# Scalsol/mega.pytorch

Hardware: AMD Instinct MI355X
Metric: frames/sec MEGA R-101 inference, 1000x600 VID clip (higher is better)
Workload: dtype bf16

## Files before the change

### include/mega_hip.h

```cpp
#ifndef MEGA_HIP_H
#define MEGA_HIP_H

#include <stddef.h>

#ifdef __cplusplus
extern "C" {
#endif

#define MEGA_F32 0
#define MEGA_BF16 1
#define MEGA_F16 2

#define MEGA_OK 0
#define MEGA_ERR_ARG 1
#define MEGA_ERR_LAUNCH 2
#define MEGA_ERR_WS 3
#define MEGA_ERR_LIMIT 4

int mega_conv2d_nhwc(const void* in, const void* w, const float* scale, const float* bias, const void* residual,
                     void* out, int N, int H, int W, int Cin, int Cout, int R, int S, int stride, int pad, int dil,
                     int relu, int ldo, int ldr, int in_dtype, int out_dtype, void* stream);
int mega_conv2d_nhwc_tile(int M, int Cout, int K);
int mega_conv2d_nhwc_plan(int M, int Cout, int K, int in_dtype);
int mega_conv2d_nhwc_plan_ex(int N, int H, int W, int Cin, int Cout, int R, int S, int stride, int pad, int dil, int ldo,
                             int has_residual, int in_dtype, int out_dtype);

size_t mega_conv2d_nhwc_workspace_bytes(int M, int Cout, int K);
int mega_conv2d_nhwc_ws(const void* in, const void* w, const float* scale, const float* bias, const void* residual,
                        void* out, int N, int H, int W, int Cin, int Cout, int R, int S, int stride, int pad, int dil,
                        int relu, int ldo, int ldr, int in_dtype, int out_dtype, void* ws, size_t ws_bytes, void* stream);

int mega_stem_conv_bn_relu(const float* in, const float* w_tap64, const float* scale, const float* bias, void* out,
                           int N, int H, int W, int out_dtype, void* stream);
int mega_stem_conv_bn_relu_bf16(const float* in, const void* w_n176_bf16, const float* scale, const float* bias,
                                void* out, int N, int H, int W, void* stream);
int mega_stem_conv_bn_relu_bf16_u8(const void* frames_u8, const void* w_n176_bf16, const float* scale, const float* bias,
                                   void* out, int N, int H, int W, float mean0, float mean1, float mean2, int to_bgr,
                                   void* stream);

int mega_stem_pool_dt(const void* in, int u8, const void* w_n176, const float* scale, const float* bias, void* out, int N,
                      int H, int W, float mean0, float mean1, float mean2, int to_bgr, int dtype, void* stream);

int mega_maxpool3x3s2_nhwc(const void* in, void* out, int N, int H, int W, int C, int dtype, void* stream);

int mega_avgpool2x2_ceil_nhwc(const void* in, void* out, int N, int H, int W, int C, int dtype, void* stream);

int mega_roi_align_fwd(const void* feat, const float* rois, void* out, int K, int C, int H, int W,
                       float spatial_scale, int pooled_h, int pooled_w, int sampling_ratio, int in_nhwc,
                       int out_nhwc, int dtype, int out_dtype, void* stream);

size_t mega_nms_full_workspace_bytes(int n);
int mega_nms(const float* dets, const float* scores, int n, float thr, int strict_gt, long long* keep_out,
             int* keep_cnt, void* ws, size_t ws_bytes, void* stream);

size_t mega_nms_workspace_bytes(int P, int nmax);
int mega_nms_sorted(const float* boxes, const int* counts, const unsigned char* valid, const int* order, int P,
                    int nmax, float thr, int strict_gt, int max_keep, int* keep_pos, int* keep_cnt,
                    unsigned char* flags, void* ws, size_t ws_bytes, void* stream);

size_t mega_rpn_select_workspace_bytes(int B, int pre_nms_top_n);
int mega_rpn_select_idx(const float* rpn_out, const float* cell_anchors, int B, int Hf, int Wf, int A, int ldc,
                        int anchor_stride, int pre_nms_top_n, int post_nms_top_n, float nms_thresh, int strict_gt,
                        float min_size, float im_w, float im_h, float* proposals, float* prop_scores, int* prop_cnt,
                        int* prop_index, void* ws, size_t ws_bytes, void* stream);

size_t mega_postprocess_workspace_bytes(int R, int NC);
int mega_postprocess(const float* logits, const float* deltas, const float* props, const int* nprop, int R, int NC,
                     float wx, float wy, float ww, float wh, float im_w, float im_h, float score_thresh,
                     float nms_thresh, int strict_gt, int max_det, float* out_boxes, float* out_scores,
                     long long* out_labels, int* out_cnt, float* probs_out, void* ws, size_t ws_bytes,
                     void* stream);

size_t mega_postprocess_batched_workspace_bytes(int B, int R, int NC);
int mega_postprocess_batched(const float* logits, const float* deltas, const float* props, const int* nprop, int B,
                             int R, int NC, float wx, float wy, float ww, float wh, float im_w, float im_h,
                             float score_thresh, float nms_thresh, int strict_gt, int max_det, float* out_boxes,
                             float* out_scores, long long* out_labels, int* out_cnt, float* probs_out, void* ws,
                             size_t ws_bytes, void* stream);

int mega_postprocess_candidates_batched(const float* logits, const float* deltas, const float* props, const int* nprop,
                                        int B, int R, int NC, float wx, float wy, float ww, float wh, float im_w,
                                        float im_h, float score_thresh, float* cboxes, float* cscores, void* stream);

size_t mega_bbox_aug_merge_workspace_bytes(int F, int K, int R, int NC);
int mega_bbox_aug_merge(const float* cboxes, const float* cscores, int F, int K, int R, int NC, const int* view_w,
                        const int* view_h, const int* view_flip, float score_thresh, float nms_thresh, int strict_gt,
                        int max_det, float* out_boxes, float* out_scores, long long* out_labels, int* out_cnt, void* ws,
                        size_t ws_bytes, void* stream);

size_t mega_soft_merge_workspace_bytes(int F, int K, int R, int NC);
int mega_soft_merge(const float* cboxes, const float* cscores, int F, int K, int R, int NC, const int* view_w,
                    const int* view_h, const int* view_flip, float score_thresh, float nms_thresh, int strict_gt,
                    int soft_method, float sigma, int vote, float vote_thresh, int vote_scoring, int max_det,
                    float* out_boxes, float* out_scores, long long* out_labels, int* out_cnt, void* ws, size_t ws_bytes,
// ... 159 lines not shown
```

### mega/pytorch_amd/_lib.py

```python
import ctypes
import os

HERE = os.path.dirname(os.path.abspath(__file__))
LIB_PATH = os.path.join(HERE, "libmega_hip.so")

c_int, c_float, c_void_p, c_size_t = ctypes.c_int, ctypes.c_float, ctypes.c_void_p, ctypes.c_size_t
c_longlong = ctypes.c_longlong

_ERR = {1: "bad argument", 2: "kernel launch failure", 3: "workspace too small", 4: "kernel loop bound exceeded"}

SIGNATURES = {
    "mega_conv2d_nhwc": (c_int, [c_void_p] * 6 + [c_int] * 15 + [c_void_p]),
    "mega_conv2d_nhwc_ws": (c_int, [c_void_p] * 6 + [c_int] * 15 + [c_void_p, c_size_t, c_void_p]),
    "mega_conv2d_nhwc_workspace_bytes": (c_size_t, [c_int] * 3),
    "mega_stem_conv_bn_relu": (c_int, [c_void_p] * 5 + [c_int] * 4 + [c_void_p]),
    "mega_stem_conv_bn_relu_bf16": (c_int, [c_void_p] * 5 + [c_int] * 3 + [c_void_p]),
    "mega_stem_conv_bn_relu_bf16_u8": (c_int, [c_void_p] * 5 + [c_int] * 3 + [c_float] * 3 + [c_int, c_void_p]),
    "mega_stem_pool_dt": (c_int, [c_void_p, c_int] + [c_void_p] * 4 + [c_int] * 3 + [c_float] * 3 + [c_int, c_int, c_void_p]),
    "mega_maxpool3x3s2_nhwc": (c_int, [c_void_p] * 2 + [c_int] * 5 + [c_void_p]),
    "mega_avgpool2x2_ceil_nhwc": (c_int, [c_void_p] * 2 + [c_int] * 5 + [c_void_p]),
    "mega_roi_align_fwd": (c_int, [c_void_p] * 3 + [c_int] * 4 + [c_float] + [c_int] * 7 + [c_void_p]),
    "mega_nms_full_workspace_bytes": (c_size_t, [c_int]),
    "mega_nms": (c_int, [c_void_p, c_void_p, c_int, c_float, c_int, c_void_p, c_void_p, c_void_p, c_size_t, c_void_p]),
    "mega_nms_workspace_bytes": (c_size_t, [c_int, c_int]),
    "mega_nms_sorted": (c_int, [c_void_p] * 4 + [c_int, c_int, c_float, c_int, c_int] + [c_void_p] * 4 +
                        [c_size_t, c_void_p]),
    "mega_rpn_select_workspace_bytes": (c_size_t, [c_int, c_int]),
    "mega_rpn_select_idx": (c_int, [c_void_p, c_void_p] + [c_int] * 8 + [c_float, c_int, c_float, c_float, c_float] +
                            [c_void_p] * 5 + [c_size_t, c_void_p]),
    "mega_postprocess_workspace_bytes": (c_size_t, [c_int, c_int]),
    "mega_postprocess": (c_int, [c_void_p] * 4 + [c_int, c_int] + [c_float] * 8 + [c_int, c_int] + [c_void_p] * 6 +
                         [c_size_t, c_void_p]),
    "mega_postprocess_batched_workspace_bytes": (c_size_t, [c_int, c_int, c_int]),
    "mega_postprocess_batched": (c_int, [c_void_p] * 4 + [c_int, c_int, c_int] + [c_float] * 8 + [c_int, c_int] +
                                 [c_void_p] * 6 + [c_size_t, c_void_p]),
    "mega_postprocess_candidates_batched": (c_int, [c_void_p] * 4 + [c_int] * 3 + [c_float] * 7 + [c_void_p] * 3),
    "mega_bbox_aug_merge_workspace_bytes": (c_size_t, [c_int] * 4),
    "mega_bbox_aug_merge": (c_int, [c_void_p, c_void_p] + [c_int] * 4 + [c_void_p] * 3 + [c_float, c_float, c_int, c_int] +
                            [c_void_p] * 5 + [c_size_t, c_void_p]),
    "mega_soft_merge_workspace_bytes": (c_size_t, [c_int] * 4),
    "mega_soft_merge": (c_int, [c_void_p, c_void_p] + [c_int] * 4 + [c_void_p] * 3 +
                        [c_float, c_float, c_int, c_int, c_float, c_int, c_float, c_int, c_int] + [c_void_p] * 5 +
                        [c_size_t, c_void_p]),
    "mega_position_logits": (c_int, [c_void_p] * 6 + [c_int] * 4 + [c_void_p]),
    "mega_relation_attention_splits": (c_int, [c_int, c_int, c_int]),
    "mega_relation_attention_workspace_bytes": (c_size_t, [c_int, c_int, c_int]),
    "mega_relation_attention": (c_int, [c_void_p, c_int, c_void_p, c_int, c_void_p, c_int, c_void_p, c_int,
                                        c_void_p, c_int, c_void_p, c_void_p, c_int, c_int, c_int, c_int, c_float,
                                        c_int, c_void_p, c_size_t, c_void_p]),
    "mega_relation_attention_batched": (c_int, [c_void_p, c_int, c_int, c_float, c_int, c_void_p]),
    "mega_position_logits_tiled_dt": (c_int, [c_void_p] * 6 + [c_int] * 3 + [c_void_p]),
    "mega_position_logits_tiled_batched_dt": (c_int, [c_void_p, c_int, c_void_p, c_void_p, c_void_p, c_int, c_void_p]),
    "mega_relation_attention_tiled_pos_dt": (c_int, [c_void_p, c_int, c_void_p, c_int, c_void_p, c_int, c_void_p,
                                                     c_void_p, c_int, c_void_p, c_void_p, c_int, c_int, c_int, c_int,
                                                     c_float, c_int, c_void_p, c_size_t, c_void_p]),
    "mega_conv2d_nhwc_tile": (c_int, [c_int] * 3),
    "mega_conv2d_nhwc_plan": (c_int, [c_int] * 4),
    "mega_conv2d_nhwc_plan_ex": (c_int, [c_int] * 14),
    "mega_preprocess_frames": (c_int, [c_void_p, c_void_p] + [c_int] * 3 + [c_float] * 3 + [c_int, c_void_p]),
    "mega_dff_warp_scale": (c_int, [c_void_p] * 4 + [c_int] * 4 + [c_void_p]),
    "mega_fgfa_pair_taps": (c_int, [c_void_p, c_longlong, c_void_p, c_longlong, c_void_p, c_void_p] + [c_int] * 4 + [c_void_p]),
    "mega_resize_bilinear_u8": (c_int, [c_void_p] * 3 + [c_int] * 5 + [c_void_p, c_void_p, c_int, c_void_p, c_void_p,
                                                                      c_int, c_void_p]),
    "mega_resize_bilinear_u8_flip": (c_int, [c_void_p] * 3 + [c_int] * 5 + [c_void_p, c_void_p, c_int, c_void_p,
                                                                           c_void_p, c_int, c_int, c_void_p]),
    "mega_fgfa_warp_aggregate": (c_int, [c_void_p] * 4 + [c_int] * 7 + [c_void_p]),
    "mega_fgfa_warp_aggregate_ring": (c_int, [c_void_p] * 4 + [c_int] * 5 + [c_void_p, c_int, c_void_p]),
    "mega_copy_segments": (c_int, [c_void_p, c_int, c_void_p]),
    "mega_bottleneck64_fwd_dt": (c_int, [c_void_p] * 11 + [c_int] * 4 + [c_void_p]),
    "mega_bottleneck64_ds_fwd_dt": (c_int, [c_void_p] * 14 + [c_int] * 4 + [c_void_p]),
    "mega_cast_f32_to_half": (c_int, [c_void_p, c_void_p, c_size_t, c_int, c_void_p]),
# ... 65 lines not shown
```

### mega/pytorch_amd/csrc/spatial.hip

```cpp
#include "common.h"

namespace {

constexpr int ST_T = 16;
constexpr int ST_P = ST_T * 2 + 5;
constexpr int ST_PW = ST_P + 1;

template <typename OT>
__global__ __launch_bounds__(256) void stem_conv_kernel(const float* __restrict__ in, const float* __restrict__ w,
                                                        const float* __restrict__ scale,
                                                        const float* __restrict__ bias, OT* __restrict__ out, int N,
                                                        int H, int W, int Ho, int Wo) {
  __shared__ float patch[3][ST_P][ST_PW];
  const int tid = threadIdx.x;
  const int n = blockIdx.z;
  const int oy0 = blockIdx.y * ST_T, ox0 = blockIdx.x * ST_T;
  const int iy0 = oy0 * 2 - 3, ix0 = ox0 * 2 - 3;
  for (int e = tid; e < 3 * ST_P * ST_P; e += 256) {
    const int c = e / (ST_P * ST_P);
    const int rem = e - c * ST_P * ST_P;
    const int y = rem / ST_P, x = rem - y * ST_P;
    const int iy = iy0 + y, ix = ix0 + x;
    float v = 0.f;
    if ((unsigned)iy < (unsigned)H && (unsigned)ix < (unsigned)W) v = in[((size_t)(n * 3 + c) * H + iy) * W + ix];
// ... 506 lines not shown
  f32x16_t acc[2][2];
#pragma unroll
  for (int i = 0; i < 2; ++i)
#pragma unroll
    for (int j = 0; j < 2; ++j)
#pragma unroll
      for (int r = 0; r < 16; ++r) acc[i][j][r] = 0.f;
#pragma unroll
  for (int ks = 0; ks < SM_K / 16; ++ks) {
    uint4 a[2], b[2];
#pragma unroll
    for (int i = 0; i < 2; ++i) {
      const unsigned* base = reinterpret_cast<const unsigned*>(
          patch + (2 * (2 * wave + i)) * SM_PS + 2 * p + (half ? stem_group_off(2 * ks + 1) : stem_group_off(2 * ks)));
      a[i] = make_uint4(base[0], base[1], base[2], base[3]);
    }
#pragma unroll
    for (int j = 0; j < 2; ++j)
      b[j] = *reinterpret_cast<const uint4*>(&wl[(j * 32 + p) * SM_WS + ks * 16 + half * 8]);
#pragma unroll
    for (int i = 0; i < 2; ++i)
#pragma unroll
      for (int j = 0; j < 2; ++j)
        acc[i][j] = __builtin_amdgcn_mfma_f32_32x32x16_bf16(__builtin_bit_cast(bf16x8_t, a[i]),
                                                            __builtin_bit_cast(bf16x8_t, b[j]), acc[i][j], 0, 0, 0);
  }
  __syncthreads();
#pragma unroll
  for (int j = 0; j < 2; ++j) {
    const int ch = j * 32 + p;
    const float sc = scale[ch], bi = bias[ch];
#pragma unroll
    for (int i = 0; i < 2; ++i) {
#pragma unroll
      for (int r = 0; r < 16; ++r) {
        const int px = (r & 3) + 8 * (r >> 2) + 4 * half;
        *reinterpret_cast<unsigned short*>(smem + ((2 * wave + i) * SM_TX + px) * SM_OUT_PS + ch * 2) =
            (bf16_t)(f32_to_bf16(fmaxf(acc[i][j][r] * sc + bi, 0.f)) & 0x7fffu);
      }
    }
  }
  __syncthreads();
#pragma unroll
  for (int i = 0; i < SM_TY * SM_TX * 8 / 256; ++i) {
    const int v = tid + 256 * i;
    const int pl = v >> 3, cv = v & 7;
    const int oy = oy0 + pl / SM_TX, ox = ox0 + pl % SM_TX;
    if (oy < Ho && ox < Wo)
      *reinterpret_cast<uint4*>(out + (((size_t)n * Ho + oy) * Wo + ox) * 64 + cv * 8) =
          *reinterpret_cast<const uint4*>(smem + pl * SM_OUT_PS + cv * 16);
  }
}

constexpr int SP_PY = 4, SP_PX = 16;
constexpr int SP_TY = 2 * SP_PY + 1, SP_TX = 2 * SP_PX + 1;
constexpr int SP_NPIX = SP_TY * SP_TX;
constexpr int SP_NBLK = (SP_NPIX + 31) / 32;
constexpr int SP_PH = 2 * SP_TY + 5, SP_PW = 2 * SP_TX + 5, SP_PS = 72;
static_assert(SP_PW + 1 <= SP_PS, "the zero-weight 8th tap reads one column past the patch");

__host__ __device__ constexpr int sp_group_off(int g) {
  const int gg = g < 21 ? g : 20;
  return (gg / 7) * (SP_PH * SP_PS) + (gg % 7) * SP_PS;
}

template <bool U8, typename HT = bf16_t>
__global__ __launch_bounds__(256, 3) void stem_pool_kernel(const void* __restrict__ in_, const bf16_t* __restrict__ w,
                                                        const float* __restrict__ scale, const float* __restrict__ bias,
                                                        bf16_t* __restrict__ out, int N, int H, int W, int Ho, int Wo, int Hp,
                                                        int Wp, float m0, float m1, float m2, int to_bgr) {
  const float* __restrict__ in = reinterpret_cast<const float*>(in_);
  const unsigned char* __restrict__ in8 = reinterpret_cast<const unsigned char*>(in_);
  constexpr int PATCH_B = (3 * SP_PH * SP_PS * 2 + 15) / 16 * 16, OUT_PS = 144;
  constexpr int LDS_B = SP_NBLK * 32 * OUT_PS > PATCH_B + 64 * SM_WS * 2 ? SP_NBLK * 32 * OUT_PS : PATCH_B + 64 * SM_WS * 2;
  __shared__ __attribute__((aligned(16))) unsigned char smem[LDS_B];
  unsigned short* patch = reinterpret_cast<unsigned short*>(smem);
  unsigned short* wl = reinterpret_cast<unsigned short*>(smem + PATCH_B);
  const int tid = threadIdx.x, lane = tid & 63, wave = tid >> 6;
  const int n = blockIdx.z;
  const int py0 = blockIdx.y * SP_PY, px0 = blockIdx.x * SP_PX;
  const int oy0 = 2 * py0 - 1, ox0 = 2 * px0 - 1;
  const int iy0 = oy0 * 2 - 3, ix0 = ox0 * 2 - 3;
  constexpr int NPL = (3 * SP_PH * SP_PS + 255) / 256, NWL = (64 * (SM_K / 8) + 255) / 256;
  float pv[NPL];
  u32x4_t wv[NWL];
#pragma unroll
  for (int i = 0; i < NPL; ++i) {
    const int e = tid + 256 * i;
    const int c = e / (SP_PH * SP_PS);
    const int rem = e - c * (SP_PH * SP_PS);
    const int y = rem / SP_PS, x = rem - y * SP_PS;
    const int iy = iy0 + y, ix = ix0 + x;
    pv[i] = 0.f;
    if (e < 3 * SP_PH * SP_PS && x < SP_PW && (unsigned)iy < (unsigned)H && (unsigned)ix < (unsigned)W) {
      if (U8) {
        const float mean = c == 0 ? m0 : (c == 1 ? m1 : m2);
        pv[i] = (float)in8[(((size_t)n * H + iy) * W + ix) * 3 + (to_bgr ? 2 - c : c)] - mean;
      } else {
        pv[i] = in[((size_t)(n * 3 + c) * H + iy) * W + ix];
      }
    }
  }
#pragma unroll
  for (int i = 0; i < NWL; ++i) {
    const int e = tid + 256 * i;
    const int row = e / (SM_K / 8), v = e - row * (SM_K / 8);
    if (e < 64 * (SM_K / 8)) wv[i] = *reinterpret_cast<const u32x4_t*>(w + row * SM_K + v * 8);
  }
#pragma unroll
  for (int i = 0; i < NPL; ++i) {
    const int e = tid + 256 * i;
    if (e < 3 * SP_PH * SP_PS) patch[e] = Half16<HT>::cvt(pv[i]);
  }
#pragma unroll
  for (int i = 0; i < NWL; ++i) {
    const int e = tid + 256 * i;
    const int row = e / (SM_K / 8), v = e - row * (SM_K / 8);
    if (e < 64 * (SM_K / 8)) *reinterpret_cast<u32x4_t*>(&wl[row * SM_WS + v * 8]) = wv[i];
  }
  __syncthreads();

  const int p = lane & 31, half = lane >> 5;
  constexpr int NB = 3;
  f32x16_t acc[NB][2];
  int pbase[NB];
#pragma unroll
  for (int b = 0; b < NB; ++b) {
    const int pix = min(32 * (wave + 4 * b) + p, SP_NPIX - 1);
    const int r = pix / SP_TX, c = pix - r * SP_TX;
    pbase[b] = 2 * r * SP_PS + 2 * c;
#pragma unroll
    for (int j = 0; j < 2; ++j)
#pragma unroll
      for (int q = 0; q < 16; ++q) acc[b][j][q] = 0.f;
  }
#pragma unroll
  for (int ks = 0; ks < SM_K / 16; ++ks) {
    u32x4_t bfr[2];
#pragma unroll
    for (int j = 0; j < 2; ++j) bfr[j] = *reinterpret_cast<const u32x4_t*>(&wl[(j * 32 + p) * SM_WS + ks * 16 + half * 8]);
#pragma unroll
    for (int b = 0; b < NB; ++b) {
      if (wave + 4 * b < SP_NBLK) {
        const unsigned* base = reinterpret_cast<const unsigned*>(patch + pbase[b] + (half ? sp_group_off(2 * ks + 1) : sp_group_off(2 * ks)));
        const u32x4_t a = {base[0], base[1], base[2], base[3]};
#pragma unroll
        for (int j = 0; j < 2; ++j) acc[b][j] = Half16<HT>::mfma32(a, bfr[j], acc[b][j]);
      }
    }
  }
  __syncthreads();
#pragma unroll
  for (int j = 0; j < 2; ++j) {
    const int ch = j * 32 + p;
    const float sc = scale[ch], bi = bias[ch];
#pragma unroll
    for (int b = 0; b < NB; ++b) {
      if (wave + 4 * b < SP_NBLK) {
#pragma unroll
        for (int q = 0; q < 16; ++q) {
          const int pix = 32 * (wave + 4 * b) + (q & 3) + 8 * (q >> 2) + 4 * half;
          const int r = pix / SP_TX, c = pix - r * SP_TX;
          const int oy = oy0 + r, ox = ox0 + c;
          const bool ok = pix < SP_NPIX && (unsigned)oy < (unsigned)Ho && (unsigned)ox < (unsigned)Wo;
          const unsigned short hv = (unsigned short)(Half16<HT>::cvt(fmaxf(acc[b][j][q] * sc + bi, 0.f)) & 0x7fffu);
          *reinterpret_cast<unsigned short*>(smem + pix * OUT_PS + ch * 2) = ok ? hv : (unsigned short)0;
        }
      }
    }
  }
  __syncthreads();
#pragma unroll
  for (int i = 0; i < SP_PY * SP_PX * 8 / 256; ++i) {
    const int v = tid + 256 * i;
    const int pl = v >> 3, cv = v & 7;
    const int ty = pl / SP_PX, tx = pl - ty * SP_PX;
    const int oy = py0 + ty, ox = px0 + tx;
    typedef unsigned short u16x8_t __attribute__((ext_vector_type(8)));
    u16x8_t m = {0, 0, 0, 0, 0, 0, 0, 0};
#pragma unroll
    for (int dy = 0; dy < 3; ++dy)
#pragma unroll
      for (int dx = 0; dx < 3; ++dx) {
        const u16x8_t q = *reinterpret_cast<const u16x8_t*>(smem + ((2 * ty + dy) * SP_TX + 2 * tx + dx) * OUT_PS + cv * 16);
        m = __builtin_elementwise_max(m, q);
      }
    if (oy < Hp && ox < Wp) *reinterpret_cast<u16x8_t*>(out + (((size_t)n * Hp + oy) * Wp + ox) * 64 + cv * 8) = m;
  }
}

}

extern "C" int mega_stem_conv_bn_relu_bf16(const float* in, const void* w_n176_bf16, const float* scale,
                                           const float* bias, void* out, int N, int H, int W, void* stream) {
  mega_clear_error();
  if (!in || !w_n176_bf16 || !scale || !bias || !out || N <= 0 || H <= 0 || W <= 0) return MEGA_ERR_ARG;
  const int Ho = (H + 6 - 7) / 2 + 1, Wo = (W + 6 - 7) / 2 + 1;
  dim3 grid(cdiv(Wo, SM_TX), cdiv(Ho, SM_TY), N);
  hipLaunchKernelGGL(stem_mfma_kernel<false>, grid, dim3(256), 0, (hipStream_t)stream, (const void*)in,
                     (const bf16_t*)w_n176_bf16, scale, bias, (bf16_t*)out, N, H, W, Ho, Wo, 0.f, 0.f, 0.f, 0);
  return mega_check_launch();
}

extern "C" int mega_stem_conv_bn_relu_bf16_u8(const void* frames_u8, const void* w_n176_bf16, const float* scale,
                                              const float* bias, void* out, int N, int H, int W, float mean0, float mean1,
                                              float mean2, int to_bgr, void* stream) {
  mega_clear_error();
  if (!frames_u8 || !w_n176_bf16 || !scale || !bias || !out || N <= 0 || H <= 0 || W <= 0) return MEGA_ERR_ARG;
  const int Ho = (H + 6 - 7) / 2 + 1, Wo = (W + 6 - 7) / 2 + 1;
  dim3 grid(cdiv(Wo, SM_TX), cdiv(Ho, SM_TY), N);
  hipLaunchKernelGGL(stem_mfma_kernel<true>, grid, dim3(256), 0, (hipStream_t)stream, frames_u8, (const bf16_t*)w_n176_bf16,
                     scale, bias, (bf16_t*)out, N, H, W, Ho, Wo, mean0, mean1, mean2, to_bgr);
  return mega_check_launch();
}

extern "C" int mega_stem_conv_bn_relu(const float* in, const float* w_tap64, const float* scale, const float* bias,
                                      void* out, int N, int H, int W, int out_dtype, void* stream) {
  mega_clear_error();
  if (!in || !w_tap64 || !scale || !bias || !out || N <= 0 || H <= 0 || W <= 0) return MEGA_ERR_ARG;
  const int Ho = (H + 6 - 7) / 2 + 1, Wo = (W + 6 - 7) / 2 + 1;
  dim3 grid(cdiv(Wo, ST_T), cdiv(Ho, ST_T), N);
  hipStream_t st = (hipStream_t)stream;
  if (out_dtype == MEGA_BF16)
    hipLaunchKernelGGL((stem_conv_kernel<bf16_t>), grid, dim3(256), 0, st, in, w_tap64, scale, bias, (bf16_t*)out, N, H,
                       W, Ho, Wo);
  else if (out_dtype == MEGA_F32)
    hipLaunchKernelGGL((stem_conv_kernel<float>), grid, dim3(256), 0, st, in, w_tap64, scale, bias, (float*)out, N, H, W,
                       Ho, Wo);
  else
    return MEGA_ERR_ARG;
  return mega_check_launch();
}

extern "C" int mega_maxpool3x3s2_nhwc(const void* in, void* out, int N, int H, int W, int C, int dtype, void* stream) {
  mega_clear_error();
  if (!in || !out || N <= 0 || H <= 0 || W <= 0 || C <= 0) return MEGA_ERR_ARG;
  const int Ho = (H + 2 - 3) / 2 + 1, Wo = (W + 2 - 3) / 2 + 1;
  hipStream_t st = (hipStream_t)stream;
  if (dtype == MEGA_BF16) {
    if (C % 8) return MEGA_ERR_ARG;
// ... 68 lines not shown
                         (float*)out, K, C, H, W, spatial_scale, pooled_h, pooled_w, sampling_ratio);
    else if (dtype == MEGA_F32)
      hipLaunchKernelGGL((roi_align_nhwc_vec_kernel<float, false>), vgrid, dim3(256), 0, st, (const float*)feat, rois,
                         (float*)out, K, C, H, W, spatial_scale, pooled_h, pooled_w, sampling_ratio);
    else
      return MEGA_ERR_ARG;
    return mega_check_launch();
  }
  dim3 grid((unsigned)(K * pooled_h * pooled_w));
  const int threads = C >= 256 ? 256 : (C >= 128 ? 128 : 64);
  if (dtype == MEGA_BF16 && out_dtype == MEGA_BF16)
    hipLaunchKernelGGL((roi_align_kernel<bf16_t, bf16_t>), grid, dim3(threads), 0, st, (const bf16_t*)feat, rois,
                       (bf16_t*)out, K, C, H, W, spatial_scale, pooled_h, pooled_w, sampling_ratio, in_nhwc, out_nhwc);
  else if (dtype == MEGA_F16 && out_dtype == MEGA_F16)
    hipLaunchKernelGGL((roi_align_kernel<f16_t, f16_t>), grid, dim3(threads), 0, st, (const f16_t*)feat, rois,
                       (f16_t*)out, K, C, H, W, spatial_scale, pooled_h, pooled_w, sampling_ratio, in_nhwc, out_nhwc);
  else if (dtype == MEGA_F32 && out_dtype == MEGA_F32)
    hipLaunchKernelGGL((roi_align_kernel<float, float>), grid, dim3(threads), 0, st, (const float*)feat, rois,
                       (float*)out, K, C, H, W, spatial_scale, pooled_h, pooled_w, sampling_ratio, in_nhwc, out_nhwc);
  else
    return MEGA_ERR_ARG;
  return mega_check_launch();
}

extern "C" int mega_avgpool2x2_ceil_nhwc(const void* in, void* out, int N, int H, int W, int C, int dtype,
                                         void* stream) {
  mega_clear_error();
  if (!in || !out || N <= 0 || H <= 0 || W <= 0 || C <= 0) return MEGA_ERR_ARG;
  const int Ho = (H + 1) / 2, Wo = (W + 1) / 2;
  hipStream_t st = (hipStream_t)stream;
  const int ve = dtype == MEGA_BF16 ? 8 : 4;
  if (C % ve) return MEGA_ERR_ARG;
  const size_t total = (size_t)N * Ho * Wo * (C / ve);
  const int blocks = (int)((total + 255) / 256 > 8192 ? 8192 : (total + 255) / 256);
  if (dtype == MEGA_BF16)
    hipLaunchKernelGGL((avgpool2_kernel<bf16_t>), dim3(blocks), dim3(256), 0, st, (const bf16_t*)in, (bf16_t*)out, N, H,
                       W, C, Ho, Wo);
  else if (dtype == MEGA_F32)
    hipLaunchKernelGGL((avgpool2_kernel<float>), dim3(blocks), dim3(256), 0, st, (const float*)in, (float*)out, N, H, W,
                       C, Ho, Wo);
  else
    return MEGA_ERR_ARG;
  return mega_check_launch();
}

extern "C" int mega_stem_pool_dt(const void* in, int u8, const void* w_n176, const float* scale, const float* bias,
                                 void* out, int N, int H, int W, float mean0, float mean1, float mean2, int to_bgr,
                                 int dtype, void* stream) {
  mega_clear_error();
  if (!in || !w_n176 || !scale || !bias || !out || N <= 0 || H <= 0 || W <= 0) return MEGA_ERR_ARG;
  if (dtype != MEGA_BF16 && dtype != MEGA_F16) return MEGA_ERR_ARG;
  const int Ho = (H + 6 - 7) / 2 + 1, Wo = (W + 6 - 7) / 2 + 1;
  const int Hp = (Ho + 2 - 3) / 2 + 1, Wp = (Wo + 2 - 3) / 2 + 1;
  dim3 grid(cdiv(Wp, SP_PX), cdiv(Hp, SP_PY), N);
  hipStream_t st = (hipStream_t)stream;
  const bf16_t* w = (const bf16_t*)w_n176;
  bf16_t* o = (bf16_t*)out;
  if (!u8) { mean0 = mean1 = mean2 = 0.f; to_bgr = 0; }
  if (dtype == MEGA_F16) {
    if (u8) hipLaunchKernelGGL((stem_pool_kernel<true, f16_t>), grid, dim3(256), 0, st, in, w, scale, bias, o, N, H, W, Ho, Wo, Hp, Wp, mean0, mean1, mean2, to_bgr);
    else hipLaunchKernelGGL((stem_pool_kernel<false, f16_t>), grid, dim3(256), 0, st, in, w, scale, bias, o, N, H, W, Ho, Wo, Hp, Wp, mean0, mean1, mean2, to_bgr);
  } else {
    if (u8) hipLaunchKernelGGL((stem_pool_kernel<true, bf16_t>), grid, dim3(256), 0, st, in, w, scale, bias, o, N, H, W, Ho, Wo, Hp, Wp, mean0, mean1, mean2, to_bgr);
    else hipLaunchKernelGGL((stem_pool_kernel<false, bf16_t>), grid, dim3(256), 0, st, in, w, scale, bias, o, N, H, W, Ho, Wo, Hp, Wp, mean0, mean1, mean2, to_bgr);
  }
  return mega_check_launch();
}

extern "C" int mega_roi_align_fwd_planes_dt(const float* feat, const float* rois, void* out, int K, int C, int H, int W,
                                            float spatial_scale, int pooled_h, int pooled_w, int sampling_ratio, int dtype,
                                            void* stream) {
  mega_clear_error();
  if (K == 0) return MEGA_OK;
  if (dtype != MEGA_BF16 && dtype != MEGA_F16) return MEGA_ERR_ARG;
  if (!feat || !rois || !out || K < 0 || C <= 0 || C % 4 || H <= 0 || W <= 0 || pooled_h <= 0 || pooled_w <= 0) return MEGA_ERR_ARG;
  const int CV = C / 4;
  const long long total = (long long)K * pooled_h * pooled_w * CV;
  const bool sliced = CV % 8 == 0 && CV / 8 >= 16 && total / 8 >= 256 * 64;
  long long nb = ((sliced ? total / 8 : total) + 255) / 256;
  if (nb > 131072) nb = 131072;
  dim3 vgrid((unsigned)(sliced ? nb * 8 : nb));
  hipStream_t st = (hipStream_t)stream;
  const bool separable = sliced && sampling_ratio <= 0 && pooled_w <= RS_MAXPW && pooled_h <= RS_MAXPW;
  if (separable) {
    if (dtype == MEGA_F16)
      hipLaunchKernelGGL((roi_align_nhwc_sep_kernel<float, 8, true, f16_t>), dim3((unsigned)(K * 8)), dim3(256), 0, st, feat, rois,
                         (float*)out, K, C, H, W, spatial_scale, pooled_h, pooled_w);
    else
      hipLaunchKernelGGL((roi_align_nhwc_sep_kernel<float, 8, true, bf16_t>), dim3((unsigned)(K * 8)), dim3(256), 0, st, feat, rois,
                         (float*)out, K, C, H, W, spatial_scale, pooled_h, pooled_w);
    return mega_check_launch();
  }
  if (dtype == MEGA_F16) {
    if (sliced)
      hipLaunchKernelGGL((roi_align_nhwc_vec_kernel<float, true, true, f16_t>), vgrid, dim3(256), 0, st, feat, rois, (float*)out, K, C,
                         H, W, spatial_scale, pooled_h, pooled_w, sampling_ratio);
    else
      hipLaunchKernelGGL((roi_align_nhwc_vec_kernel<float, false, true, f16_t>), vgrid, dim3(256), 0, st, feat, rois, (float*)out, K,
                         C, H, W, spatial_scale, pooled_h, pooled_w, sampling_ratio);
  } else if (sliced)
    hipLaunchKernelGGL((roi_align_nhwc_vec_kernel<float, true, true>), vgrid, dim3(256), 0, st, feat, rois, (float*)out, K, C, H,
                       W, spatial_scale, pooled_h, pooled_w, sampling_ratio);
  else
    hipLaunchKernelGGL((roi_align_nhwc_vec_kernel<float, false, true>), vgrid, dim3(256), 0, st, feat, rois, (float*)out, K, C, H,
                       W, spatial_scale, pooled_h, pooled_w, sampling_ratio);
  return mega_check_launch();
}
```

### mega/pytorch_amd/ops.py

```python
import contextlib
import ctypes
import threading
import math

import torch

from . import _lib

F32, BF16, F16 = 0, 1, 2
_DT = {torch.float32: F32, torch.bfloat16: BF16, torch.float16: F16}
_HALF = (torch.bfloat16, torch.float16)


def _dt(t):
    try:
        return _DT[t.dtype]
    except KeyError:
        raise TypeError("unsupported dtype %s (float32 / bfloat16 / float16 only)" % t.dtype)


_LAUNCH = threading.local()


def _stream():
# ... 291 lines not shown
    out = torch.empty((N, Ho, Wo, 64), dtype=out_dtype, device=x_nchw.device)
    _tok = _pb("stem", 2.0 * N * Ho * Wo * 64 * 147, x_nchw.numel() * 4 + out.numel() * out.element_size())
    if out_dtype == torch.bfloat16 and w_n160 is not None:
        _gpu(w_n160)
        assert w_n160.dtype == torch.bfloat16 and tuple(w_n160.shape) == (64, 176) and w_n160.is_contiguous()
        rc = lib.mega_stem_conv_bn_relu_bf16(_ptr(x_nchw), _ptr(w_n160), _ptr(scale), _ptr(bias), _ptr(out), N, H, W,
                                             _stream())
    else:
        rc = lib.mega_stem_conv_bn_relu(_ptr(x_nchw), _ptr(w_tap64), _ptr(scale), _ptr(bias), _ptr(out), N, H, W,
                                        _DT[out_dtype], _stream())
    _pe(_tok)
    _lib.check(rc, "mega_stem_conv_bn_relu")
    return out


def stem_u8(frames_u8, w_n160, scale, bias, mean, to_bgr=True):
    _gpu(frames_u8, w_n160, scale, bias)
    lib = _lib.load()
    N, H, W, C = frames_u8.shape
    assert C == 3 and frames_u8.dtype == torch.uint8 and frames_u8.is_contiguous()
    assert w_n160.dtype == torch.bfloat16 and tuple(w_n160.shape) == (64, 176) and w_n160.is_contiguous()
    Ho, Wo = (H - 1) // 2 + 1, (W - 1) // 2 + 1
    out = torch.empty((N, Ho, Wo, 64), dtype=torch.bfloat16, device=frames_u8.device)
    _tok = _pb("stem", 2.0 * N * Ho * Wo * 64 * 147, frames_u8.numel() + out.numel() * 2)
    rc = lib.mega_stem_conv_bn_relu_bf16_u8(_ptr(frames_u8), _ptr(w_n160), _ptr(scale), _ptr(bias), _ptr(out), N, H, W,
                                            float(mean[0]), float(mean[1]), float(mean[2]), int(to_bgr), _stream())
    _pe(_tok)
    _lib.check(rc, "mega_stem_conv_bn_relu_bf16_u8")
    return out


def stem_pool(x, w_n160, scale, bias, mean=None, to_bgr=True):
    _gpu(x, w_n160, scale, bias)
    lib = _lib.load()
    u8 = x.dtype == torch.uint8
    if u8:
        N, H, W, C = x.shape
        assert mean is not None
    else:
        N, C, H, W = x.shape
        assert x.dtype == torch.float32
        mean = (0.0, 0.0, 0.0)
    assert C == 3 and x.is_contiguous()
    assert w_n160.dtype in _HALF and tuple(w_n160.shape) == (64, 176) and w_n160.is_contiguous()
    Ho, Wo = (H - 1) // 2 + 1, (W - 1) // 2 + 1
    Hp, Wp = (Ho - 1) // 2 + 1, (Wo - 1) // 2 + 1
    out = torch.empty((N, Hp, Wp, 64), dtype=w_n160.dtype, device=x.device)
    _tok = _pb("stem", 2.0 * N * Ho * Wo * 64 * 147, x.numel() * x.element_size() + out.numel() * 2)
    rc = lib.mega_stem_pool_dt(_ptr(x), int(u8), _ptr(w_n160), _ptr(scale), _ptr(bias), _ptr(out), N, H, W,
                               float(mean[0]), float(mean[1]), float(mean[2]), int(to_bgr), _dt(w_n160), _stream())
    _pe(_tok)
    _lib.check(rc, "mega_stem_pool_dt")
    return out


def pack_stem_weight_bf16(w_oihw, dtype=torch.bfloat16):
    w = torch.zeros((64, 22, 8), dtype=torch.float32, device=w_oihw.device)
    w[:, :21, :7] = w_oihw.detach().float().reshape(64, 21, 7)
    w = w.reshape(64, 176)
    return w.to(dtype).contiguous()


def maxpool3x3s2(x):
    _gpu(x)
    lib = _lib.load()
    N, H, W, C = x.shape
    assert x.is_contiguous()
    Ho, Wo = (H - 1) // 2 + 1, (W - 1) // 2 + 1
    out = torch.empty((N, Ho, Wo, C), dtype=x.dtype, device=x.device)
    _tok = _pb("maxpool", 0.0, (x.numel() + out.numel()) * x.element_size())
    rc = lib.mega_maxpool3x3s2_nhwc(_ptr(x), _ptr(out), N, H, W, C, _dt(x), _stream())
    _pe(_tok)
    _lib.check(rc, "mega_maxpool3x3s2_nhwc")
    return out


def roi_align(feat, rois, spatial_scale, pooled, sampling_ratio, in_nhwc=True, out_nhwc=True):
    _gpu(feat, rois)
    lib = _lib.load()
    if in_nhwc:
        B, H, W, C = feat.shape
    else:
        B, C, H, W = feat.shape
    ph, pw = pooled
    K = rois.shape[0]
    assert feat.is_contiguous() and rois.dtype == torch.float32 and rois.is_contiguous() and rois.shape[1] == 5
    shape = (K, ph * pw, C) if out_nhwc else (K, C, ph, pw)
    out = torch.empty(shape, dtype=feat.dtype, device=feat.device)
    _tok = _pb("roi_align", 0.0, out.numel() * out.element_size() + feat.numel() * feat.element_size())
    rc = lib.mega_roi_align_fwd(_ptr(feat), _ptr(rois), _ptr(out), K, C, H, W, float(spatial_scale), ph, pw,
                                int(sampling_ratio), int(in_nhwc), int(out_nhwc), _dt(feat), _dt(feat), _stream())
    _pe(_tok)
    _lib.check(rc, "mega_roi_align_fwd")
    return out


def roi_align_planes(feat, rois, spatial_scale, pooled, sampling_ratio, dtype=torch.bfloat16):
    _gpu(feat, rois)
    lib = _lib.load()
    B, H, W, C = feat.shape
    ph, pw = pooled
    K = rois.shape[0]
    assert feat.dtype == torch.float32 and feat.is_contiguous() and rois.dtype == torch.float32 and rois.is_contiguous()
    assert rois.shape[1] == 5 and C % 4 == 0
    out = torch.empty((K, 2 * ph * pw * C), dtype=dtype, device=feat.device)
    _tok = _pb("roi_align", 0.0, out.numel() * 2 + feat.numel() * 4)
# ... 1009 lines not shown
```

Baseline: 903.4.

## Make fused stem conv+maxpool kernel persistent with register-resident weights and vectorized u8 loads

The stem conv+BN+ReLU+maxpool kernel becomes a persistent grid-stride kernel sized to twice the CU count. The weight fragments and scale/bias are loaded once per block, with the weights kept in registers instead of being restaged in LDS for every tile. The u8 input path now loads 4-pixel runs as 12-byte vectors, the tile shape changes to 7x12, and the epilogue writes packed channel vectors into a separate LDS staging area. The trade-offs are more registers, occupancy dropping from 3 to 2 blocks per SIMD, more dynamic LDS, and more halo overlap from the new tile shape.

```diff
diff --git a/include/mega_hip.h b/include/mega_hip.h
--- a/include/mega_hip.h
+++ b/include/mega_hip.h
@@ -40,6 +40,7 @@
 
 int mega_stem_pool_dt(const void* in, int u8, const void* w_n176, const float* scale, const float* bias, void* out, int N,
                       int H, int W, float mean0, float mean1, float mean2, int to_bgr, int dtype, void* stream);
+void mega_stem_pool_tile(int* rows, int* cols);
 
 int mega_maxpool3x3s2_nhwc(const void* in, void* out, int N, int H, int W, int C, int dtype, void* stream);
 
diff --git a/mega/pytorch_amd/_lib.py b/mega/pytorch_amd/_lib.py
--- a/mega/pytorch_amd/_lib.py
+++ b/mega/pytorch_amd/_lib.py
@@ -17,6 +17,7 @@
     "mega_stem_conv_bn_relu_bf16": (c_int, [c_void_p] * 5 + [c_int] * 3 + [c_void_p]),
     "mega_stem_conv_bn_relu_bf16_u8": (c_int, [c_void_p] * 5 + [c_int] * 3 + [c_float] * 3 + [c_int, c_void_p]),
     "mega_stem_pool_dt": (c_int, [c_void_p, c_int] + [c_void_p] * 4 + [c_int] * 3 + [c_float] * 3 + [c_int, c_int, c_void_p]),
+    "mega_stem_pool_tile": (None, [c_void_p, c_void_p]),
     "mega_maxpool3x3s2_nhwc": (c_int, [c_void_p] * 2 + [c_int] * 5 + [c_void_p]),
     "mega_avgpool2x2_ceil_nhwc": (c_int, [c_void_p] * 2 + [c_int] * 5 + [c_void_p]),
     "mega_roi_align_fwd": (c_int, [c_void_p] * 3 + [c_int] * 4 + [c_float] + [c_int] * 7 + [c_void_p]),
diff --git a/mega/pytorch_amd/csrc/spatial.hip b/mega/pytorch_amd/csrc/spatial.hip
--- a/mega/pytorch_amd/csrc/spatial.hip
+++ b/mega/pytorch_amd/csrc/spatial.hip
@@ -582,140 +582,206 @@
   }
 }
 
-constexpr int SP_PY = 4, SP_PX = 16;
+constexpr int SP_PY = 7, SP_PX = 12;
 constexpr int SP_TY = 2 * SP_PY + 1, SP_TX = 2 * SP_PX + 1;
 constexpr int SP_NPIX = SP_TY * SP_TX;
 constexpr int SP_NBLK = (SP_NPIX + 31) / 32;
-constexpr int SP_PH = 2 * SP_TY + 5, SP_PW = 2 * SP_TX + 5, SP_PS = 72;
+constexpr int SP_NB = SP_NBLK / 4;
+static_assert(SP_NBLK % 4 == 0, "the four waves share the row blocks evenly");
+constexpr int SP_PH = 2 * SP_TY + 5, SP_PW = 2 * SP_TX + 5, SP_PS = 56;
 static_assert(SP_PW + 1 <= SP_PS, "the zero-weight 8th tap reads one column past the patch");
+static_assert(SP_PS % 4 == 0, "a patch row is filled in runs of 4 pixels");
+constexpr int SP_NGX = SP_PS / 4, SP_NG = SP_PH * SP_NGX;
+constexpr int SP_GPT = (SP_NG + 255) / 256;
+constexpr int SP_OUT_PS = 144;
+constexpr int SP_PATCH_B = 3 * SP_PH * SP_PS * 2, SP_STAGE_B = SP_NBLK * 32 * SP_OUT_PS;
+static_assert(SP_PATCH_B % 16 == 0 && SP_STAGE_B % 16 == 0, "16-byte LDS vectors");
+constexpr int SP_LDS = SP_PATCH_B + SP_STAGE_B + 128 * 4;
 
 __host__ __device__ constexpr int sp_group_off(int g) {
   const int gg = g < 21 ? g : 20;
   return (gg / 7) * (SP_PH * SP_PS) + (gg % 7) * SP_PS;
 }
 
+typedef unsigned int u32x3_t __attribute__((ext_vector_type(3)));
+
+__device__ __forceinline__ void sp_load_run(const unsigned char* __restrict__ in8, int n, int iy, int ix, int H, int W, bool active,
+                                            u32x3_t& raw, unsigned& mask) {
+  raw = u32x3_t{0u, 0u, 0u};
+  mask = 0u;
+  if (active && (unsigned)iy < (unsigned)H) {
+    const unsigned char* row = in8 + ((size_t)n * H + iy) * (size_t)W * 3;
+    if (ix >= 0 && ix + 3 < W) {
+      __builtin_memcpy(&raw, row + (ptrdiff_t)ix * 3, 12);
+      mask = 0xfu;
+    } else {
+#pragma unroll
+      for (int k = 0; k < 4; ++k) {
+        if ((unsigned)(ix + k) < (unsigned)W) {
+          mask |= 1u << k;
+#pragma unroll
+          for (int s = 0; s < 3; ++s) {
+            const int q = 3 * k + s;
+            raw[q >> 2] |= (unsigned)row[(ptrdiff_t)(ix + k) * 3 + s] << (8 * (q & 3));
+          }
+        }
+      }
+    }
+  }
+}
+
 template <bool U8, typename HT = bf16_t>
-__global__ __launch_bounds__(256, 3) void stem_pool_kernel(const void* __restrict__ in_, const bf16_t* __restrict__ w,
+__global__ __launch_bounds__(256, 2) void stem_pool_kernel(const void* __restrict__ in_, const bf16_t* __restrict__ w,
                                                         const float* __restrict__ scale, const float* __restrict__ bias,
                                                         bf16_t* __restrict__ out, int N, int H, int W, int Ho, int Wo, int Hp,
-                                                        int Wp, float m0, float m1, float m2, int to_bgr) {
+                                                        int Wp, float m0, float m1, float m2, int to_bgr, int tiles_y,
+                                                        int tiles_x, int ntiles) {
   const float* __restrict__ in = reinterpret_cast<const float*>(in_);
   const unsigned char* __restrict__ in8 = reinterpret_cast<const unsigned char*>(in_);
-  constexpr int PATCH_B = (3 * SP_PH * SP_PS * 2 + 15) / 16 * 16, OUT_PS = 144;
-  constexpr int LDS_B = SP_NBLK * 32 * OUT_PS > PATCH_B + 64 * SM_WS * 2 ? SP_NBLK * 32 * OUT_PS : PATCH_B + 64 * SM_WS * 2;
-  __shared__ __attribute__((aligned(16))) unsigned char smem[LDS_B];
-  unsigned short* patch = reinterpret_cast<unsigned short*>(smem);
-  unsigned short* wl = reinterpret_cast<unsigned short*>(smem + PATCH_B);
+  extern __shared__ __attribute__((aligned(16))) unsigned char sp_smem[];
+  unsigned short* patch = reinterpret_cast<unsigned short*>(sp_smem);
+  unsigned char* stage = sp_smem + SP_PATCH_B;
+  float* sb = reinterpret_cast<float*>(sp_smem + SP_PATCH_B + SP_STAGE_B);
   const int tid = threadIdx.x, lane = tid & 63, wave = tid >> 6;
-  const int n = blockIdx.z;
-  const int py0 = blockIdx.y * SP_PY, px0 = blockIdx.x * SP_PX;
-  const int oy0 = 2 * py0 - 1, ox0 = 2 * px0 - 1;
-  const int iy0 = oy0 * 2 - 3, ix0 = ox0 * 2 - 3;
-  constexpr int NPL = (3 * SP_PH * SP_PS + 255) / 256, NWL = (64 * (SM_K / 8) + 255) / 256;
-  float pv[NPL];
-  u32x4_t wv[NWL];
-#pragma unroll
-  for (int i = 0; i < NPL; ++i) {
-    const int e = tid + 256 * i;
-    const int c = e / (SP_PH * SP_PS);
-    const int rem = e - c * (SP_PH * SP_PS);
-    const int y = rem / SP_PS, x = rem - y * SP_PS;
-    const int iy = iy0 + y, ix = ix0 + x;
-    pv[i] = 0.f;
-    if (e < 3 * SP_PH * SP_PS && x < SP_PW && (unsigned)iy < (unsigned)H && (unsigned)ix < (unsigned)W) {
-      if (U8) {
-        const float mean = c == 0 ? m0 : (c == 1 ? m1 : m2);
-        pv[i] = (float)in8[(((size_t)n * H + iy) * W + ix) * 3 + (to_bgr ? 2 - c : c)] - mean;
-      } else {
-        pv[i] = in[((size_t)(n * 3 + c) * H + iy) * W + ix];
-      }
-    }
-  }
-#pragma unroll
-  for (int i = 0; i < NWL; ++i) {
-    const int e = tid + 256 * i;
-    const int row = e / (SM_K / 8), v = e - row * (SM_K / 8);
-    if (e < 64 * (SM_K / 8)) wv[i] = *reinterpret_cast<const u32x4_t*>(w + row * SM_K + v * 8);
-  }
-#pragma unroll
-  for (int i = 0; i < NPL; ++i) {
-    const int e = tid + 256 * i;
-    if (e < 3 * SP_PH * SP_PS) patch[e] = Half16<HT>::cvt(pv[i]);
-  }
-#pragma unroll
-  for (int i = 0; i < NWL; ++i) {
-    const int e = tid + 256 * i;
-    const int row = e / (SM_K / 8), v = e - row * (SM_K / 8);
-    if (e < 64 * (SM_K / 8)) *reinterpret_cast<u32x4_t*>(&wl[row * SM_WS + v * 8]) = wv[i];
-  }
-  __syncthreads();
-
   const int p = lane & 31, half = lane >> 5;
-  constexpr int NB = 3;
-  f32x16_t acc[NB][2];
-  int pbase[NB];
-#pragma unroll
-  for (int b = 0; b < NB; ++b) {
+
+  u32x4_t wf[2][SM_K / 16];
+#pragma unroll
+  for (int j = 0; j < 2; ++j)
+#pragma unroll
+    for (int ks = 0; ks < SM_K / 16; ++ks)
+      wf[j][ks] = *reinterpret_cast<const u32x4_t*>(w + (j * 32 + p) * SM_K + ks * 16 + half * 8);
+  if (tid < 64) {
+    sb[tid] = scale[tid];
+    sb[64 + tid] = bias[tid];
+  }
+  int pbase[SP_NB], prc[SP_NB];
+#pragma unroll
+  for (int b = 0; b < SP_NB; ++b) {
     const int pix = min(32 * (wave + 4 * b) + p, SP_NPIX - 1);
     const int r = pix / SP_TX, c = pix - r * SP_TX;
     pbase[b] = 2 * r * SP_PS + 2 * c;
-#pragma unroll
-    for (int j = 0; j < 2; ++j)
-#pragma unroll
-      for (int q = 0; q < 16; ++q) acc[b][j][q] = 0.f;
-  }
-#pragma unroll
-  for (int ks = 0; ks < SM_K / 16; ++ks) {
-    u32x4_t bfr[2];
-#pragma unroll
-    for (int j = 0; j < 2; ++j) bfr[j] = *reinterpret_cast<const u32x4_t*>(&wl[(j * 32 + p) * SM_WS + ks * 16 + half * 8]);
-#pragma unroll
-    for (int b = 0; b < NB; ++b) {
-      if (wave + 4 * b < SP_NBLK) {
-        const unsigned* base = reinterpret_cast<const unsigned*>(patch + pbase[b] + (half ? sp_group_off(2 * ks + 1) : sp_group_off(2 * ks)));
+    prc[b] = (r << 16) | c;
+  }
+  int gy[SP_GPT], gx4[SP_GPT];
+#pragma unroll
+  for (int i = 0; i < SP_GPT; ++i) {
+    const int g = tid + 256 * i;
+    gy[i] = g / SP_NGX;
+    gx4[i] = 4 * (g - gy[i] * SP_NGX);
+  }
+  const float ms[3] = {to_bgr ? m2 : m0, m1, to_bgr ? m0 : m2};
+  const int plane[3] = {to_bgr ? 2 * SP_PH * SP_PS : 0, SP_PH * SP_PS, to_bgr ? 0 : 2 * SP_PH * SP_PS};
+  const int tiles_per_image = tiles_y * tiles_x;
+
+  for (int t = blockIdx.x; t < ntiles; t += gridDim.x) {
+    const int n = t / tiles_per_image, rem = t - n * tiles_per_image;
+    const int ty = rem / tiles_x, tx = rem - ty * tiles_x;
+    const int py0 = ty * SP_PY, px0 = tx * SP_PX;
+    const int oy0 = 2 * py0 - 1, ox0 = 2 * px0 - 1;
+    const int iy0 = oy0 * 2 - 3, ix0 = ox0 * 2 - 3;
+    if (U8) {
+      u32x3_t raw[SP_GPT];
+      unsigned mask[SP_GPT];
+#pragma unroll
+      for (int i = 0; i < SP_GPT; ++i)
+        sp_load_run(in8, n, iy0 + gy[i], ix0 + gx4[i], H, W, tid + 256 * i < SP_NG, raw[i], mask[i]);
+#pragma unroll
+      for (int i = 0; i < SP_GPT; ++i) {
+        if (tid + 256 * i < SP_NG) {
+#pragma unroll
+          for (int s = 0; s < 3; ++s) {
+            float f[4];
+#pragma unroll
+            for (int k = 0; k < 4; ++k) {
+              const int q = 3 * k + s;
+              const float v = (float)((raw[i][q >> 2] >> (8 * (q & 3))) & 0xffu) - ms[s];
+              f[k] = (mask[i] >> k) & 1u ? v : 0.f;
+            }
+            typedef unsigned int u32x2_t __attribute__((ext_vector_type(2)));
+            *reinterpret_cast<u32x2_t*>(patch + plane[s] + gy[i] * SP_PS + gx4[i]) =
+                u32x2_t{Half16<HT>::pack2(f[0], f[1]), Half16<HT>::pack2(f[2], f[3])};
+          }
+        }
+      }
+    } else {
+      constexpr int NE = 3 * SP_PH * SP_PS;
+#pragma unroll 1
+      for (int e0 = tid; e0 < NE; e0 += 256 * 8) {
+        float pv[8];
+#pragma unroll
+        for (int i = 0; i < 8; ++i) {
+          const int e = e0 + 256 * i;
+          const int c = e / (SP_PH * SP_PS);
+          const int r2 = e - c * (SP_PH * SP_PS);
+          const int y = r2 / SP_PS, x = r2 - y * SP_PS;
+          const int iy = iy0 + y, ix = ix0 + x;
+          pv[i] = 0.f;
+          if (e < NE && x < SP_PW && (unsigned)iy < (unsigned)H && (unsigned)ix < (unsigned)W)
+            pv[i] = in[((size_t)(n * 3 + c) * H + iy) * W + ix];
+        }
+#pragma unroll
+        for (int i = 0; i < 8; ++i) {
+          const int e = e0 + 256 * i;
+          if (e < NE) patch[e] = Half16<HT>::cvt(pv[i]);
+        }
+      }
+    }
+    __syncthreads();
+
+#pragma unroll
+    for (int b = 0; b < SP_NB; ++b) {
+      f32x16_t acc[2];
+#pragma unroll
+      for (int j = 0; j < 2; ++j)
+#pragma unroll
+        for (int q = 0; q < 16; ++q) acc[j][q] = 0.f;
+#pragma unroll
+      for (int ks = 0; ks < SM_K / 16; ++ks) {
+        const int dk = sp_group_off(2 * ks + 1) - sp_group_off(2 * ks);
+        const unsigned* base = reinterpret_cast<const unsigned*>(patch + (pbase[b] + (half ? dk : 0)) + sp_group_off(2 * ks));
         const u32x4_t a = {base[0], base[1], base[2], base[3]};
 #pragma unroll
-        for (int j = 0; j < 2; ++j) acc[b][j] = Half16<HT>::mfma32(a, bfr[j], acc[b][j]);
-      }
-    }
-  }
-  __syncthreads();
-#pragma unroll
-  for (int j = 0; j < 2; ++j) {
-    const int ch = j * 32 + p;
-    const float sc = scale[ch], bi = bias[ch];
-#pragma unroll
-    for (int b = 0; b < NB; ++b) {
-      if (wave + 4 * b < SP_NBLK) {
-#pragma unroll
-        for (int q = 0; q < 16; ++q) {
-          const int pix = 32 * (wave + 4 * b) + (q & 3) + 8 * (q >> 2) + 4 * half;
-          const int r = pix / SP_TX, c = pix - r * SP_TX;
-          const int oy = oy0 + r, ox = ox0 + c;
-          const bool ok = pix < SP_NPIX && (unsigned)oy < (unsigned)Ho && (unsigned)ox < (unsigned)Wo;
-          const unsigned short hv = (unsigned short)(Half16<HT>::cvt(fmaxf(acc[b][j][q] * sc + bi, 0.f)) & 0x7fffu);
-          *reinterpret_cast<unsigned short*>(smem + pix * OUT_PS + ch * 2) = ok ? hv : (unsigned short)0;
+        for (int j = 0; j < 2; ++j) acc[j] = Half16<HT>::mfma32(wf[j][ks], a, acc[j]);
+      }
+      const int pix = 32 * (wave + 4 * b) + p;
+      const int oy = oy0 + (prc[b] >> 16), ox = ox0 + (prc[b] & 0xffff);
+      const bool ok = (unsigned)oy < (unsigned)Ho && (unsigned)ox < (unsigned)Wo;
+#pragma unroll
+      for (int j = 0; j < 2; ++j) {
+#pragma unroll
+        for (int g = 0; g < 4; ++g) {
+          const int ch0 = 32 * j + 8 * g + 4 * half;
+          const f32x4_t sc = *reinterpret_cast<const f32x4_t*>(sb + ch0), bi = *reinterpret_cast<const f32x4_t*>(sb + 64 + ch0);
+          float v[4];
+#pragma unroll
+          for (int i = 0; i < 4; ++i) v[i] = fmaxf(acc[j][4 * g + i] * sc[i] + bi[i], 0.f);
+          const unsigned lo = Half16<HT>::pack2(v[0], v[1]) & 0x7fff7fffu, hi = Half16<HT>::pack2(v[2], v[3]) & 0x7fff7fffu;
+          typedef unsigned int u32x2_t __attribute__((ext_vector_type(2)));
+          *reinterpret_cast<u32x2_t*>(stage + pix * SP_OUT_PS + ch0 * 2) = ok ? u32x2_t{lo, hi} : u32x2_t{0u, 0u};
         }
       }
     }
-  }
-  __syncthreads();
-#pragma unroll
-  for (int i = 0; i < SP_PY * SP_PX * 8 / 256; ++i) {
-    const int v = tid + 256 * i;
-    const int pl = v >> 3, cv = v & 7;
-    const int ty = pl / SP_PX, tx = pl - ty * SP_PX;
-    const int oy = py0 + ty, ox = px0 + tx;
-    typedef unsigned short u16x8_t __attribute__((ext_vector_type(8)));
-    u16x8_t m = {0, 0, 0, 0, 0, 0, 0, 0};
-#pragma unroll
-    for (int dy = 0; dy < 3; ++dy)
-#pragma unroll
-      for (int dx = 0; dx < 3; ++dx) {
-        const u16x8_t q = *reinterpret_cast<const u16x8_t*>(smem + ((2 * ty + dy) * SP_TX + 2 * tx + dx) * OUT_PS + cv * 16);
-        m = __builtin_elementwise_max(m, q);
-      }
-    if (oy < Hp && ox < Wp) *reinterpret_cast<u16x8_t*>(out + (((size_t)n * Hp + oy) * Wp + ox) * 64 + cv * 8) = m;
+    __syncthreads();
+#pragma unroll
+    for (int i = 0; i < (SP_PY * SP_PX * 8 + 255) / 256; ++i) {
+      const int v = tid + 256 * i;
+      const int pl = v >> 3, cv = v & 7;
+      const int yy = pl / SP_PX, xx = pl - yy * SP_PX;
+      const int oy = py0 + yy, ox = px0 + xx;
+      if (v < SP_PY * SP_PX * 8) {
+        typedef unsigned short u16x8_t __attribute__((ext_vector_type(8)));
+        u16x8_t m = {0, 0, 0, 0, 0, 0, 0, 0};
+#pragma unroll
+        for (int dy = 0; dy < 3; ++dy)
+#pragma unroll
+          for (int dx = 0; dx < 3; ++dx) {
+            const u16x8_t q = *reinterpret_cast<const u16x8_t*>(stage + ((2 * yy + dy) * SP_TX + 2 * xx + dx) * SP_OUT_PS + cv * 16);
+            m = __builtin_elementwise_max(m, q);
+          }
+        if (oy < Hp && ox < Wp) *reinterpret_cast<u16x8_t*>(out + (((size_t)n * Hp + oy) * Wp + ox) * 64 + cv * 8) = m;
+      }
+    }
   }
 }
 
@@ -890,19 +956,47 @@
   if (dtype != MEGA_BF16 && dtype != MEGA_F16) return MEGA_ERR_ARG;
   const int Ho = (H + 6 - 7) / 2 + 1, Wo = (W + 6 - 7) / 2 + 1;
   const int Hp = (Ho + 2 - 3) / 2 + 1, Wp = (Wo + 2 - 3) / 2 + 1;
-  dim3 grid(cdiv(Wp, SP_PX), cdiv(Hp, SP_PY), N);
+  const int tiles_y = cdiv(Hp, SP_PY), tiles_x = cdiv(Wp, SP_PX);
+  const long tiles = (long)N * tiles_y * tiles_x;
+  if (tiles > 0x7FFF0000L) return MEGA_ERR_ARG;
+  if (u8 && (size_t)H * W * 3 > 0x7FFFFFFFu) return MEGA_ERR_ARG;
+  int cus = 256;
+  {
+    static int cached[64] = {0};
+    int dev = 0, n = 0;
+    if (hipGetDevice(&dev) != hipSuccess || dev < 0 || dev >= 64) dev = 0;
+    if (!cached[dev]) {
+      if (hipDeviceGetAttribute(&n, hipDeviceAttributeMultiprocessorCount, dev) == hipSuccess && n > 0) cached[dev] = n;
+      else cached[dev] = 256;
+    }
+    cus = cached[dev];
+  }
+  const dim3 grid((unsigned)(tiles < 2L * cus ? tiles : 2L * cus));
+  const int nt = (int)tiles;
   hipStream_t st = (hipStream_t)stream;
   const bf16_t* w = (const bf16_t*)w_n176;
   bf16_t* o = (bf16_t*)out;
   if (!u8) { mean0 = mean1 = mean2 = 0.f; to_bgr = 0; }
+#define MEGA_SP_LAUNCH(U8_, HT_)                                                                                           \
+  do {                                                                                                                     \
+    (void)hipFuncSetAttribute((const void*)stem_pool_kernel<U8_, HT_>, hipFuncAttributeMaxDynamicSharedMemorySize, SP_LDS); \
+    hipLaunchKernelGGL((stem_pool_kernel<U8_, HT_>), grid, dim3(256), SP_LDS, st, in, w, scale, bias, o, N, H, W, Ho, Wo,   \
+                       Hp, Wp, mean0, mean1, mean2, to_bgr, tiles_y, tiles_x, nt);                                         \
+  } while (0)
   if (dtype == MEGA_F16) {
-    if (u8) hipLaunchKernelGGL((stem_pool_kernel<true, f16_t>), grid, dim3(256), 0, st, in, w, scale, bias, o, N, H, W, Ho, Wo, Hp, Wp, mean0, mean1, mean2, to_bgr);
-    else hipLaunchKernelGGL((stem_pool_kernel<false, f16_t>), grid, dim3(256), 0, st, in, w, scale, bias, o, N, H, W, Ho, Wo, Hp, Wp, mean0, mean1, mean2, to_bgr);
+    if (u8) MEGA_SP_LAUNCH(true, f16_t);
+    else MEGA_SP_LAUNCH(false, f16_t);
   } else {
-    if (u8) hipLaunchKernelGGL((stem_pool_kernel<true, bf16_t>), grid, dim3(256), 0, st, in, w, scale, bias, o, N, H, W, Ho, Wo, Hp, Wp, mean0, mean1, mean2, to_bgr);
-    else hipLaunchKernelGGL((stem_pool_kernel<false, bf16_t>), grid, dim3(256), 0, st, in, w, scale, bias, o, N, H, W, Ho, Wo, Hp, Wp, mean0, mean1, mean2, to_bgr);
-  }
+    if (u8) MEGA_SP_LAUNCH(true, bf16_t);
+    else MEGA_SP_LAUNCH(false, bf16_t);
+  }
+#undef MEGA_SP_LAUNCH
   return mega_check_launch();
+}
+
+extern "C" void mega_stem_pool_tile(int* rows, int* cols) {
+  if (rows) *rows = SP_PY;
+  if (cols) *cols = SP_PX;
 }
 
 extern "C" int mega_roi_align_fwd_planes_dt(const float* feat, const float* rois, void* out, int K, int C, int H, int W,
diff --git a/mega/pytorch_amd/ops.py b/mega/pytorch_amd/ops.py
--- a/mega/pytorch_amd/ops.py
+++ b/mega/pytorch_amd/ops.py
@@ -367,6 +367,12 @@
     _pe(_tok)
     _lib.check(rc, "mega_stem_pool_dt")
     return out
+
+
+def stem_pool_tile():
+    th, tw = ctypes.c_int(0), ctypes.c_int(0)
+    _lib.load().mega_stem_pool_tile(ctypes.byref(th), ctypes.byref(tw))
+    return th.value, tw.value
 
 
 def pack_stem_weight_bf16(w_oihw, dtype=torch.bfloat16):
```

Result: faster. 916.5, median of 6 (+1.5%).
